# microsoft/Sora

Measured on AMD Instinct MI355X. Metric: IQ Msamples/s through 802.11a 54 Mbps RX PHY, higher is better.
Workload: dtype int16 IQ / u8 path metrics

## Files before the change

### sora_amd/csrc/dev_vit16.h

```cpp
#pragma once
#include <hip/hip_runtime.h>
#include "kernels.h"
#include "dev_viterbi.h"

namespace sora {
namespace {

template <int WIN, int LOOK> struct Geom16 {
    static constexpr int kMaxWalk = (WIN + LOOK + 7) / 8 + 2;
    static constexpr int P = kMaxWalk;
    static constexpr int kPathBytes = 40;
};

template <int WIN, int LOOK> struct Lds16 {
    uint16_t ring[Geom16<WIN, LOOK>::P][4][64];
    union {
        uint32_t udump[4][64];
        uint16_t ops[4][24][2];
        uint16_t ops2[2][4][24][2];
    };
    uint32_t path[8][Geom16<WIN, LOOK>::kPathBytes / 4];
};

constexpr unsigned kW[4] = { 0u, 21u, 42u, 63u };

__device__ __forceinline__ unsigned v_of_lane(unsigned l)
{
    const unsigned b0 = l & 1u, b1 = (l >> 1) & 1u, b2 = (l >> 2) & 1u, b3 = (l >> 3) & 1u;
    const unsigned c3 = b2, c1 = b3, c0 = b0 ^ c3, c2 = b1 ^ c3;
    return c0 | (c1 << 1) | (c2 << 2) | (c3 << 3);
}
__device__ __forceinline__ unsigned lane_of_v(unsigned v)
{
    const unsigned c0 = v & 1u, c1 = (v >> 1) & 1u, c2 = (v >> 2) & 1u, c3 = (v >> 3) & 1u;
    return c0 ^ (c2 << 1) ^ (c1 << 3) ^ (c3 ? 7u : 0u);
}
__device__ __forceinline__ unsigned rev6u(unsigned x) { return __brev(x) >> 26; }

template <int CTRL> __device__ __forceinline__ unsigned dppx(unsigned v) { return (unsigned)__builtin_amdgcn_update_dpp(0, (int)v, CTRL, 0xF, 0xF, true); }

__device__ __forceinline__ unsigned partner(unsigned v, int ph)
{
    switch (ph) {
    case 0: return dppx<0x140>(v);
    case 1: return dppx<0x1B>(v);
    case 2: return dppx<0x141>(v);
    case 3: return dppx<0x4E>(v);
    case 4: return dppx<0x128>(v);
    default: return dppx<0xB1>(v);
    }
}

struct Vit16 {
    unsigned U[4];
    unsigned MX[24];
    unsigned MY[6];
    unsigned sadr[3][4];
};

template <int WHICH, int P>
__device__ __forceinline__ void acs16(Vit16& V, int t24, unsigned a, unsigned b, unsigned pos512[3])
{
    const int ph = t24 % 6, k = t24 % 8;
    const unsigned Kp = (WHICH == 0 ? 14u : 7u) * kFld + (kOne << k);
    unsigned bm;
    if (WHICH == 0)      bm = (a ^ V.MX[t24]) + (b ^ V.MY[ph]);
    else if (WHICH == 1) bm = a ^ V.MX[t24];
    else                 bm = b ^ V.MX[t24];
    const unsigned bo = Kp - bm;
    const int rx = ph == 0 ? 2 : ph == 1 ? 1 : 0;
    unsigned N[4];
#pragma unroll
    for (int i = 0; i < 4; i++) {
        const unsigned X = V.U[i], Y = partner(V.U[i ^ rx], ph);
        const bool wb = (kW[i] >> (5 - ph)) & 1u;
        N[i] = wb ? pk_min16(X + bo, Y + bm) : pk_min16(X + bm, Y + bo);
    }
#pragma unroll
    for (int i = 0; i < 4; i++) V.U[i] = N[i];
    if (k == 7) {
        const int jb = t24 / 8;
#pragma unroll
        for (int i = 0; i < 4; i++) {
            const unsigned w = bank_word(V.U[i]);
            const unsigned addr = V.sadr[jb][i] + pos512[jb];
            asm volatile("ds_write_b16 %0, %1" : : "v"(addr), "v"(w) : "memory");
            V.U[i] &= 0xFE00FE00u;
        }
    }
}

__device__ __forceinline__ unsigned row_min_u32(unsigned v)
{
    v = min(v, dppx<0xB1>(v)); v = min(v, dppx<0x4E>(v)); v = min(v, dppx<0x141>(v)); v = min(v, dppx<0x128>(v));
    return v;
}
__device__ __forceinline__ unsigned row_pkmin(unsigned v)
{
    v = pk_min16(v, dppx<0xB1>(v)); v = pk_min16(v, dppx<0x4E>(v)); v = pk_min16(v, dppx<0x141>(v)); v = pk_min16(v, dppx<0x128>(v));
    return v;
}
__device__ __forceinline__ unsigned wave_min_u32(unsigned v) { return (unsigned)__builtin_amdgcn_readfirstlane((int)dpp_min_u32_wave(v)); }
__device__ __forceinline__ unsigned wave_max_u32(unsigned v) { return ~wave_min_u32(~v); }

template <int CR, int WIN, int LOOK, int BITS>
struct Forward16 {
    static constexpr int P = Geom16<WIN, LOOK>::P, GB = Puncture<CR>::GB, GS = Puncture<CR>::GS, CW = Puncture<CR>::CW;
    static constexpr int NV = Puncture<CR>::NV;
    struct Chunk { uint32_t v[CW]; };
    struct Raw { SoftRaw r[NV]; };

    Vit16 V;
    unsigned row, half;
    uint32_t my_j;
    SoftCursor<BITS, CW> cur[NV];
    uint32_t my_base;
    const uint8_t* soft;
    uint16_t* my_ops;
    const uint4* row_ops;
    uint32_t pos;
    unsigned pos512[3];
    uint32_t tr, nsteps;
    uint32_t next_thr;
    bool all_done;

    __device__ __forceinline__ void init(Lds16<WIN, LOOK>& S, const uint8_t* __restrict__ soft_, uint32_t my_soft_off, uint32_t my_first, uint32_t my_last, unsigned start,
                                         uint32_t nsteps_)
    {
        const unsigned lane = threadIdx.x & 63, l16 = lane & 15;
        row = lane >> 4; half = lane & 1u;
        const unsigned v0 = v_of_lane(l16);
        nsteps = nsteps_;
#pragma unroll
        for (int i = 0; i < 4; i++) V.U[i] = (v0 ^ kW[i]) == 0 ? 0u : start;
        const unsigned ring_base = (unsigned)(uintptr_t)&S.ring[0][0][0];
#pragma unroll
        for (int jb = 0; jb < 3; jb++)
#pragma unroll
            for (int i = 0; i < 4; i++) V.sadr[jb][i] = ring_base + ((row * 64u + rev6u(rol6(v0 ^ kW[i], jb == 0 ? 2 : jb == 1 ? 4 : 0))) << 1);
#pragma unroll
        for (int t = 0; t < 24; t++) {
            const int ph = t % 6, k = t % 8;
            const unsigned n = rol6(v0, ph + 1);
            const bool vb = (v0 >> (5 - ph)) & 1u;
            const unsigned ma = (__popc(n & 0155) & 1) ? 7u * kFld : 0u, mb = (__popc(n & 0117) & 1) ? 7u * kFld : 0u;
            const unsigned mx = Puncture<CR>::which_of(ph) == 2 ? mb : ma;
            V.MX[t] = vb ? ((mx ^ (7u * kFld)) | (kOne << k)) : mx;
            if (t < 6) V.MY[t] = vb ? (mb ^ (7u * kFld)) : mb;
        }
        tr = 0; pos = 0;
        my_j = l16 >> 1;
#pragma unroll
        for (int v = 0; v < NV; v++) cur[v].init(my_soft_off, my_first + my_j + 8u * v, my_last);
        my_base = my_soft_off + my_first + my_j;
        soft = soft_;
        my_ops = &S.ops[row][my_j][half];
        row_ops = reinterpret_cast<const uint4*>(&S.ops[row][0][0]);
        set_row_pos();
        clear_ops(S);
    }
    __device__ __forceinline__ bool going() const { return tr < nsteps && !all_done; }

    __device__ __forceinline__ void normalize()
    {
        const unsigned m = row_pkmin(pk_min16(pk_min16(V.U[0], V.U[1]), pk_min16(V.U[2], V.U[3])));
#pragma unroll
        for (int i = 0; i < 4; i++) V.U[i] -= m;
    }
    static __device__ __forceinline__ uint32_t pos_of(uint32_t p, int jb) { const uint32_t q = p + 512u * (uint32_t)jb; return min(q, q - 512u * (uint32_t)P); }
    __device__ __forceinline__ void set_row_pos()
    {
        pos512[0] = pos; pos512[1] = pos_of(pos, 1); pos512[2] = pos_of(pos512[1], 1);
    }
    __device__ __forceinline__ void end_row() { pos = pos_of(pos512[2], 1); set_row_pos(); }
    __device__ __forceinline__ Raw fetch(uint32_t c) const
    {
        Raw R;
#pragma unroll
        for (int v = 0; v < NV; v++) R.r[v] = cur[v].fetch(soft, c);
        return R;
    }
    __device__ __forceinline__ void put(const Raw& R, uint16_t* mine) const
    {
#pragma unroll
        for (int v = 0; v < NV; v++) soft_put(mine + 16 * v, cur[v], R.r[v]);
    }
    __device__ __forceinline__ void clear_ops(Lds16<WIN, LOOK>& S) const
    {
        if constexpr (BITS == kSoftScaled) {
            static_assert(sizeof(S.ops2) == 3 * 64 * 4, "three dwords per lane");
            uint32_t* z = reinterpret_cast<uint32_t*>(&S.ops2[0][0][0][0]) + (threadIdx.x & 63);
            z[0] = 0u; z[64] = 0u; z[128] = 0u;
            lds_fence();
        }
    }
    __device__ __forceinline__ uint32_t fast_base(uint32_t c0) const { return my_base + c0 * (uint32_t)CW; }
    template <int DC> __device__ __forceinline__ Raw fetch_at(uint32_t p) const
    {
        static_assert(BITS == kSoftScaled, "one byte per value");
        Raw R;
#pragma unroll
        for (int v = 0; v < NV; v++) { R.r[v].sh = 0; R.r[v].w = soft[(size_t)p + (size_t)(DC * CW + 8 * v)]; }
        return R;
    }
    static __device__ __forceinline__ Chunk get(const uint4* table)
    {
        Chunk K;
#pragma unroll
        for (int i = 0; i < (CW + 3) / 4; i++) {
            const uint4 x = table[i];
            K.v[4 * i] = x.x; K.v[4 * i + 1] = x.y;
            if (4 * i + 2 < CW) { K.v[4 * i + 2] = x.z; K.v[4 * i + 3] = x.w; }
        }
        return K;
    }
    __device__ __forceinline__ Chunk unpack(const Raw& R) const
    {
        put(R, my_ops);
        lds_fence();
        const Chunk K = get(row_ops);
        lds_fence();
        return K;
    }
    __device__ __forceinline__ void group(const Chunk& K, int h, int i0)
    {
        const int k0 = i0 / GS * GB, t24 = 12 * h + i0;
        acs16<0, P>(V, t24, K.v[k0], K.v[k0 + 1], pos512);
        if (CR != 0) acs16<1, P>(V, t24 + 1, K.v[k0 + 2], 0, pos512);
        if (CR == 2) acs16<2, P>(V, t24 + 2, 0, K.v[k0 + 3], pos512);
        if ((t24 + GS) % 8 == 0) normalize();
    }
    __device__ __forceinline__ void fast_chunk(const Chunk& K, int h)
    {
#pragma unroll
        for (int g = 0; g < 12 / GS; g++) group(K, h, g * GS);
        tr += 12;
    }
    template <typename CHECK> __device__ __forceinline__ void slow_chunk(const Chunk& K, int h, CHECK& check)
    {
#pragma unroll
        for (int g = 0; g < 12 / GS; g++) {
            if (going()) {
                group(K, h, g * GS);
                tr += GS;
                check(12 * h + g * GS + GS - 1);
            }
        }
    }
    template <typename CHECK> __device__ __forceinline__ void chunk(const Chunk& K, int h, CHECK& check)
    {
        if (tr + 12 <= nsteps && next_thr > tr + 12) fast_chunk(K, h); else slow_chunk(K, h, check);
    }
};

template <int WIN, int LOOK, bool LANE_OB = false>
__device__ __noinline__ void trace16(unsigned lds_off, unsigned U0, unsigned U1, unsigned U2, unsigned U3, uint32_t tr_, uint32_t ob_, uint32_t pj_, uint32_t k_,
                                     uint32_t my_cnt, uint8_t* my_out)
{
    using G = Geom16<WIN, LOOK>;
    constexpr int P = G::P, K = G::kMaxWalk;
    constexpr int NR = K - 1, NF = NR / 4, NW = K / 4 + 1;
    static_assert(NR % 4 == 0 || NR % 4 == 2, "the walk's words are packed in pairs");
    static_assert(NW * 4 <= G::kPathBytes && NW >= WIN / 32 + 1, "the stream's registers hold a window and fit Lds16::path");
    typedef __attribute__((address_space(3))) Lds16<WIN, LOOK> lds_t;
    typedef __attribute__((address_space(3))) const uint16_t lds_u16;
    lds_t& S = *(lds_t*)(uintptr_t)lds_off;
    auto uni = [](uint32_t v) { return (uint32_t)__builtin_amdgcn_readfirstlane((int)v); };
    const uint32_t tr = uni(tr_), ob = LANE_OB ? ob_ : uni(ob_), pj = uni(pj_), k = uni(k_);
    const unsigned lane = threadIdx.x & 63, row = lane >> 4, l16 = lane & 15, half = lane & 1u;
    const unsigned v0 = v_of_lane(l16);
    const unsigned U[4] = { U0, U1, U2, U3 };
    const uint32_t j = (tr - 1) >> 3, nn = tr - 8u * j, m_lo = ob >> 3;
    const unsigned rowbase = (unsigned)(uintptr_t)&S.ring[0][row][0], sh = 8u * half;
    auto ring_j = [&](unsigned idx) -> unsigned { return *(lds_u16*)(uintptr_t)(rowbase + pj + (idx << 1)); };
#pragma unroll
    for (int i = 0; i < 4; i++) S.udump[i][lane] = U[i];
    lds_fence();
    unsigned key[2] = { 0xFFFFFFFFu, 0xFFFFFFFFu };
#pragma unroll
    for (int i = 0; i < 4; i++) {
        const unsigned st = rol6(v0 ^ kW[i], tr);
        unsigned lastA, lastB;
        if (k == 7) { const unsigned w = ring_j(rev6u(st)); lastA = (w >> 7) & 1u; lastB = (w >> 15) & 1u; }
        else { lastA = (U[i] >> k) & 1u; lastB = (U[i] >> (17 + k)) & 1u; }
        const unsigned mA = ((U[i] & 0xFFFFu) >> 9 << 1) | lastA, mB = (U[i] >> 25 << 1) | lastB;
        key[0] = min(key[0], (mA << 8) | (st << 2)); key[1] = min(key[1], (mB << 8) | (st << 2));
    }
    const unsigned kA = row_min_u32(key[0]), kB = row_min_u32(key[1]);
    const unsigned st = ((half ? kB : kA) >> 2) & 0x3Fu;
    const unsigned s0 = rol6(st, 6u - tr % 6u);
    const unsigned b4 = (s0 >> 4) & 1u, b5 = (s0 >> 5) & 1u;
    const unsigned ri = b4 | (b5 << 1);
    const unsigned sl = lane_of_v((s0 ^ (b4 ? 21u : 0u) ^ (b5 ? 42u : 0u)) & 15u);
    const unsigned Ust = S.udump[ri][row * 16u + sl];
    unsigned H;
    if (nn == 8) H = (ring_j(rev6u(st)) >> sh) & 0xFFu;
    else H = ((Ust >> (17u * half)) & 0xFFu) & ((1u << nn) - 1u);
    unsigned q = rev6u(((st >> nn) | rev6u(H & 0x3Fu)) & 0x3Fu);
    unsigned pr[NR / 2];
    uint32_t p = pj;
#pragma unroll
    for (int i = 1; i < K; i++) {
        uint32_t d;
        p = __builtin_sub_overflow(p, 512u, &d) ? 512u * (uint32_t)(P - 1) : d;
        unsigned base = rowbase + p;
        asm volatile("" : "+v"(base));
        const unsigned raw = *(lds_u16*)(uintptr_t)(base + (q << 1));
        q = __builtin_amdgcn_ubfe(raw, sh, 6u);
        const int s = K - 1 - i;
        if (s & 1) pr[s >> 1] = raw << 16; else pr[s >> 1] |= raw;
    }
    unsigned R[NW];
    const unsigned sel = 0x06040200u + 0x01010101u * half;
#pragma unroll
    for (int w = 0; w < NF; w++) R[w] = __builtin_amdgcn_perm(pr[2 * w + 1], pr[2 * w], sel);
    if (NR % 4 == 0) R[NF] = H;
    else R[NF] = __builtin_amdgcn_perm(H, pr[2 * NF], 0x0C040200u + 0x00000101u * half);
    const uint32_t sfirst = (uint32_t)(K - 1) - (j - m_lo);
    bool fast = !LANE_OB;
    if (!LANE_OB) {
        const bool whole = my_cnt == (uint32_t)WIN && sfirst == 1u && (((uintptr_t)my_out + m_lo) & 3u) == 0;
        fast = __ballot(!(whole || my_cnt == 0)) == 0;
    }
    if (fast) {
        if (my_cnt != 0 && l16 < 2) {
            uint32_t* o = reinterpret_cast<uint32_t*>(my_out + m_lo);
#pragma unroll
            for (int dw = 0; dw < WIN / 32; dw++) o[dw] = __builtin_amdgcn_alignbit(R[dw + 1], R[dw], 14);
        }
    } else {
        __attribute__((address_space(3))) uint32_t* pw = S.path[row * 2u + half];
        if (l16 < 2) {
#pragma unroll
            for (int w = 0; w < NW; w++) pw[w] = R[w];
        }
        lds_fence();
        __attribute__((address_space(3))) const uint8_t* pth = (__attribute__((address_space(3))) const uint8_t*)pw;
        const uint32_t nbytes = my_cnt >> 3;
        for (uint32_t z = l16 >> 1; z < nbytes; z += 8) {
            const uint32_t sb = sfirst + z;
            my_out[m_lo + z] = (uint8_t)(((unsigned)pth[sb] >> 6) | (((unsigned)pth[sb + 1] & 0x3Fu) << 2));
        }
    }
    lds_fence();
}

}
}
```

### sora_amd/csrc/k_vit16.hip

```cpp
#include <hip/hip_runtime.h>

#include "dev_vit16.h"

namespace sora {

namespace {

template <int CR, int WIN, int LOOK, int BITS>
__device__ __forceinline__ void forward16(Lds16<WIN, LOOK>& S, const uint8_t* __restrict__ soft, uint32_t my_soft_off, uint32_t my_nsoft,
                                          uint32_t nstepsA, uint32_t nstepsB, uint32_t my_tr_end, bool my_valid, uint8_t* my_out)
{
    using F16 = Forward16<CR, WIN, LOOK, BITS>;
    using Chunk = typename F16::Chunk;
    using Raw = typename F16::Raw;
    constexpr int GS = F16::GS;
    F16 F;
    F.init(S, soft, my_soft_off, 0, max(my_nsoft, 1u) - 1u, 0x18u * kFld, wave_max_u32(max(nstepsA, nstepsB)));

    uint32_t ob = 0;
    bool my_done = !my_valid;

    auto trace = [&](uint32_t my_cnt, int t24_last) {
        trace16<WIN, LOOK>((unsigned)(uintptr_t)&S, F.V.U[0], F.V.U[1], F.V.U[2], F.V.U[3], F.tr, ob, F16::pos_of(F.pos, t24_last / 8), (uint32_t)(t24_last % 8), my_cnt, my_out);
    };
    auto next_event = [&]() -> uint32_t {
        const uint32_t mine = my_done ? kNever : my_tr_end;
        return min(ob + (uint32_t)(WIN + LOOK + 6), wave_min_u32(mine));
    };
    F.next_thr = next_event();
    F.all_done = wave_min_u32(my_done ? 1u : 0u) != 0u;
    auto check = [&](int t24_last) {
        if (F.tr >= F.next_thr) {
            const bool partial = F.tr >= ob + (uint32_t)(WIN + LOOK + 6);
            uint32_t cnt = 0;
            if (!my_done) {
                if (F.tr >= my_tr_end) { cnt = my_tr_end - ob - 6; my_done = true; }
                else if (partial) cnt = WIN;
            }
            if (wave_max_u32(cnt) != 0u) { trace(cnt, t24_last); F.clear_ops(S); }
            if (partial) ob += WIN;
            F.next_thr = next_event();
            F.all_done = wave_min_u32(my_done ? 1u : 0u) != 0u;
        }
    };

    uint16_t* my_ops2[2] = { &S.ops2[0][F.row][F.my_j][F.half], &S.ops2[1][F.row][F.my_j][F.half] };
    const uint4* row_ops2[2] = { reinterpret_cast<const uint4*>(&S.ops2[0][F.row][0][0]), reinterpret_cast<const uint4*>(&S.ops2[1][F.row][0][0]) };
    auto stage = [&](const Raw& R, int t) { F.put(R, my_ops2[t]); };
    auto collect = [&](int t) -> Chunk { lds_fence(); return F16::get(row_ops2[t]); };
    auto fast_chunk_mid = [&](const Chunk& K, int h, Chunk& Knext, int tnext) {
#pragma unroll
        for (int g = 0; g < 12 / GS; g++) {
            if (g == (12 / GS) / 2) Knext = collect(tnext);
            F.group(K, h, g * GS);
        }
        F.tr += 12;
    };

    uint32_t c = 0;
    Raw b0 = F.fetch(0), b1 = F.fetch(1), b2, b3;
    while (F.going()) {
        const uint32_t lim = min(F.nsteps, F.next_thr - 1);
        uint32_t rows = lim > F.tr ? (lim - F.tr) / 24 : 0;
        if (rows >= 2) {
            Chunk Ka, Kb;
            b2 = F.fetch(c + 2);
            stage(b0, 0); Ka = collect(0); lds_fence();
            if constexpr (BITS == kSoftScaled) {
                uint32_t p = F.fast_base(c);
                for (; rows >= 2; rows -= 2) {
                    b3 = F.template fetch_at<3>(p); stage(b1, 1); fast_chunk_mid(Ka, 0, Kb, 1);
                    b0 = F.template fetch_at<4>(p); stage(b2, 0); fast_chunk_mid(Kb, 1, Ka, 0);
                    F.end_row();
                    b1 = F.template fetch_at<5>(p); stage(b3, 1); fast_chunk_mid(Ka, 0, Kb, 1);
                    b2 = F.template fetch_at<6>(p); stage(b0, 0); fast_chunk_mid(Kb, 1, Ka, 0);
                    F.end_row();
                    c += 4; p += 4u * (uint32_t)F16::CW;
                }
            } else {
                for (; rows >= 2; rows -= 2) {
                    b3 = F.fetch(c + 3); stage(b1, 1); fast_chunk_mid(Ka, 0, Kb, 1);
                    b0 = F.fetch(c + 4); stage(b2, 0); fast_chunk_mid(Kb, 1, Ka, 0);
                    F.end_row();
                    b1 = F.fetch(c + 5); stage(b3, 1); fast_chunk_mid(Ka, 0, Kb, 1);
                    b2 = F.fetch(c + 6); stage(b0, 0); fast_chunk_mid(Kb, 1, Ka, 0);
                    F.end_row();
                    c += 4;
                }
            }
            lds_fence();
        }
        if (!(F.tr < F.nsteps)) break;
        b2 = F.fetch(c + 2);
        if (rows) F.fast_chunk(F.unpack(b0), 0); else F.chunk(F.unpack(b0), 0, check);
        if (!F.going()) break;
        b3 = F.fetch(c + 3);
        if (rows) F.fast_chunk(F.unpack(b1), 1); else F.chunk(F.unpack(b1), 1, check);
        F.end_row();
        b0 = b2; b1 = b3;
        c += 2;
    }
}

template <int WIN, int LOOK, int BITS>
__device__ __forceinline__ void viterbi16_body(const VitJob* __restrict__ jobs, const uint32_t* __restrict__ njobs3, uint32_t njobs_single, uint32_t stride,
                                               const uint8_t* __restrict__ soft, uint8_t* __restrict__ out)
{
    __shared__ Lds16<WIN, LOOK> S;
    uint32_t n[3] = { njobs_single, 0, 0 };
    if (njobs3) { n[0] = njobs3[0]; n[1] = njobs3[1]; n[2] = njobs3[2]; }
    uint32_t w = uni(blockIdx.x), list = 0;
    while (list < 3 && w >= (n[list] + 7) / 8) { w -= (n[list] + 7) / 8; list++; }
    if (list >= 3) return;
    const uint32_t njobs = uni(n[list]);
    jobs += (size_t)list * stride;
    const unsigned lane = threadIdx.x & 63, row = lane >> 4, half = lane & 1u;
    const uint32_t fa = 8u * w + 2u * row, fb = fa + 1u;
    const bool hasA = fa < njobs, hasB = fb < njobs;
    const VitJob& GA = jobs[hasA ? fa : 8u * w];
    const VitJob& GBj = jobs[hasB ? fb : (hasA ? fa : 8u * w)];
    const uint32_t code_rate = uni(jobs[8u * w].code_rate);
    const uint32_t gsd = code_rate == 0 ? 2u : code_rate == 2 ? 4u : 3u, gss = code_rate == 0 ? 1u : code_rate == 2 ? 3u : 2u;
    const uint32_t nstepsA = hasA ? GA.nsoft / gsd * gss : 0u, nstepsB = hasB ? GBj.nsoft / gsd * gss : 0u;
    const VitJob& Mine = half ? GBj : GA;
    const bool my_valid = half ? hasB : hasA;
    const uint32_t my_tr_end = Mine.length * 8u + 16u + 6u;
    uint8_t* my_out = out + Mine.out_off;
    if (code_rate == 0)      forward16<0, WIN, LOOK, BITS>(S, soft, Mine.soft_off, Mine.nsoft, nstepsA, nstepsB, my_tr_end, my_valid, my_out);
    else if (code_rate == 1) forward16<1, WIN, LOOK, BITS>(S, soft, Mine.soft_off, Mine.nsoft, nstepsA, nstepsB, my_tr_end, my_valid, my_out);
    else                     forward16<2, WIN, LOOK, BITS>(S, soft, Mine.soft_off, Mine.nsoft, nstepsA, nstepsB, my_tr_end, my_valid, my_out);
}

}

__global__ void __launch_bounds__(64) k_viterbi16(const VitJob* __restrict__ jobs, const uint32_t* __restrict__ njobs3, uint32_t njobs_single, uint32_t stride,
        const uint8_t* __restrict__ soft, uint8_t* __restrict__ out)
{ viterbi16_body<256, 24, kSoftScaled>(jobs, njobs3, njobs_single, stride, soft, out); }
__global__ void __launch_bounds__(64) k_viterbi16_p3(const VitJob* __restrict__ jobs, const uint32_t* __restrict__ njobs3, uint32_t njobs_single, uint32_t stride,
        const uint8_t* __restrict__ soft, uint8_t* __restrict__ out)
{ viterbi16_body<256, 24, 3>(jobs, njobs3, njobs_single, stride, soft, out); }
__global__ void __launch_bounds__(64) k_viterbi16_11n(const VitJob* __restrict__ jobs, const uint32_t* __restrict__ njobs3, uint32_t njobs_single,
        uint32_t stride, const uint8_t* __restrict__ soft, uint8_t* __restrict__ out)
{ viterbi16_body<192, 36, 8>(jobs, njobs3, njobs_single, stride, soft, out); }

}
```

### sora_amd/csrc/rx_types.h

```cpp
#pragma once
#include <stdint.h>

namespace sora {

struct CapDesc {
    uint64_t offset;
    uint32_t nsamples;
    uint32_t capture_id;
    uint32_t slot_base;
    uint32_t nslots;
};

struct FrameRow {
    uint32_t capture;
    uint32_t start_sample;
    uint32_t end_sample;
    uint32_t error_code;
    uint32_t rate_kbps;
    uint16_t length, nsym;
    uint16_t code_rate, nbpsc;
    uint32_t slot0;
    uint32_t crc32;
    int16_t  cfo_est;
    int16_t  cfo_comp, sfo_comp, cfo_tracker, sfo_tracker;
    uint16_t valid;
    uint32_t data_start;
    uint32_t pad[3];
};

struct FrameCtx {
    uint32_t freq[64];
    uint32_t chan[64];
};

struct VitJob {
    uint32_t soft_off;
    uint32_t nsoft;
    uint32_t length;
    uint32_t dec_off;
    uint32_t out_off;
    uint32_t valid;
    uint32_t code_rate;
    uint32_t soft_bits;
};

constexpr int kWinWarm = 144;
constexpr int kWinVecBytes = 256;
constexpr unsigned kWinStatBanks = 64;

struct TrackRec {
    int16_t cfo_comp, sfo_comp;
    int16_t avg, del;
};

struct JobRef { uint32_t list, idx; bool ok; };
__host__ __device__ inline JobRef locate_job(uint32_t g, const uint32_t* njobs)
{
    JobRef r; r.ok = true;
    const uint32_t n0 = njobs[0], n1 = njobs[1], n2 = njobs[2];
    if (g < n0) { r.list = 0; r.idx = g; }
    else if (g < n0 + n1) { r.list = 1; r.idx = g - n0; }
    else if (g < n0 + n1 + n2) { r.list = 2; r.idx = g - n0 - n1; }
    else { r.list = 0; r.idx = 0; r.ok = false; }
    return r;
}

constexpr int kSoftPerSlot = 288;
constexpr int kSoftBytesPerSlot = 288;
constexpr int kSoftSlack = 64;
constexpr int kSoftScaled = 9;
constexpr int kSoftPad = 66 * 1024;
static_assert(kSoftPad >= 65568 + 7 * 24 + 16 + kSoftSlack, "the pad holds a maximal stream and the look-ahead");
constexpr int kOutPerSlot  = 32;

constexpr uint32_t E_FRAME_OK = 0x00000001u, E_PLCP_HEADER_FAIL = 0x80000005u, E_CRC32_FAIL = 0x80000006u,
                   E_CS_TIMEOUT = 0x80000007u,
                   E_INTERNAL_TIMEOUT = 0x8000F001u;

}
```

Before: 56640.

## Distribute soft bits by DPP row broadcast instead of LDS staging in Viterbi

For the one-byte soft path, each lane now loads a dword of soft bits directly from global memory. Lanes swap bytes with a DPP quad permute, then each ACS step pulls its branch-metric operand from the owning lane with a DPP row broadcast. This removes the LDS put/fence/get staging and the clearing of the ops buffer from the hot trellis loop. The cost is extra permute and broadcast instructions per ACS step, and a larger look-ahead pad requirement.

```diff
diff --git a/sora_amd/csrc/dev_vit16.h b/sora_amd/csrc/dev_vit16.h
--- a/sora_amd/csrc/dev_vit16.h
+++ b/sora_amd/csrc/dev_vit16.h
@@ -38,6 +38,19 @@
 __device__ __forceinline__ unsigned rev6u(unsigned x) { return __brev(x) >> 26; }
 
 template <int CTRL> __device__ __forceinline__ unsigned dppx(unsigned v) { return (unsigned)__builtin_amdgcn_update_dpp(0, (int)v, CTRL, 0xF, 0xF, true); }
+__device__ __forceinline__ unsigned row_bcast(unsigned v, int n)
+{
+    switch (n) {
+    case 0: return dppx<0x150>(v);
+    case 2: return dppx<0x152>(v);
+    case 4: return dppx<0x154>(v);
+    case 6: return dppx<0x156>(v);
+    case 8: return dppx<0x158>(v);
+    case 10: return dppx<0x15A>(v);
+    case 12: return dppx<0x15C>(v);
+    default: return dppx<0x15E>(v);
+    }
+}
 
 __device__ __forceinline__ unsigned partner(unsigned v, int ph)
 {
@@ -103,12 +116,26 @@
 __device__ __forceinline__ unsigned wave_min_u32(unsigned v) { return (unsigned)__builtin_amdgcn_readfirstlane((int)dpp_min_u32_wave(v)); }
 __device__ __forceinline__ unsigned wave_max_u32(unsigned v) { return ~wave_min_u32(~v); }
 
-template <int CR, int WIN, int LOOK, int BITS>
+template <int CR, int WIN, int LOOK, int BITS, bool BCAST = false>
 struct Forward16 {
     static constexpr int P = Geom16<WIN, LOOK>::P, GB = Puncture<CR>::GB, GS = Puncture<CR>::GS, CW = Puncture<CR>::CW;
     static constexpr int NV = Puncture<CR>::NV;
-    struct Chunk { uint32_t v[CW]; };
+    static constexpr int RB = 2 * CW, RD = RB / 4, NS = (RD + 7) / 8;
+    static_assert(!BCAST || (BITS == kSoftScaled && RB % 4 == 0), "one byte per value, rows of whole dwords");
+    struct Chunk {
+        uint32_t v[CW];
+        __device__ __forceinline__ unsigned op(int, int k) const { return v[k]; }
+    };
     struct Raw { SoftRaw r[NV]; };
+    struct RawRow { uint32_t d[NS]; };
+    struct Row {
+        uint32_t r[NS][4];
+        __device__ __forceinline__ unsigned op(int h, int k) const
+        {
+            const int kk = h * CW + k;
+            return row_bcast(r[kk >> 5][kk & 3], 2 * ((kk >> 2) & 7));
+        }
+    };
 
     Vit16 V;
     unsigned row, half;
@@ -152,12 +179,12 @@
         my_j = l16 >> 1;
 #pragma unroll
         for (int v = 0; v < NV; v++) cur[v].init(my_soft_off, my_first + my_j + 8u * v, my_last);
-        my_base = my_soft_off + my_first + my_j;
+        my_base = BCAST ? my_soft_off + 4u * my_j : my_soft_off + my_first + my_j;
         soft = soft_;
         my_ops = &S.ops[row][my_j][half];
         row_ops = reinterpret_cast<const uint4*>(&S.ops[row][0][0]);
         set_row_pos();
-        clear_ops(S);
+        if constexpr (!BCAST) clear_ops(S);
     }
     __device__ __forceinline__ bool going() const { return tr < nsteps && !all_done; }
 
@@ -194,15 +221,6 @@
             lds_fence();
         }
     }
-    __device__ __forceinline__ uint32_t fast_base(uint32_t c0) const { return my_base + c0 * (uint32_t)CW; }
-    template <int DC> __device__ __forceinline__ Raw fetch_at(uint32_t p) const
-    {
-        static_assert(BITS == kSoftScaled, "one byte per value");
-        Raw R;
-#pragma unroll
-        for (int v = 0; v < NV; v++) { R.r[v].sh = 0; R.r[v].w = soft[(size_t)p + (size_t)(DC * CW + 8 * v)]; }
-        return R;
-    }
     static __device__ __forceinline__ Chunk get(const uint4* table)
     {
         Chunk K;
@@ -222,21 +240,40 @@
         lds_fence();
         return K;
     }
-    __device__ __forceinline__ void group(const Chunk& K, int h, int i0)
+    __device__ __forceinline__ uint32_t row_base(uint32_t row_index) const { return my_base + row_index * (uint32_t)RB; }
+    template <int DR> __device__ __forceinline__ RawRow fetch_row(uint32_t p) const
+    {
+        RawRow R;
+#pragma unroll
+        for (int s = 0; s < NS; s++) R.d[s] = *reinterpret_cast<const uint32_t*>(soft + ((size_t)p + (size_t)(DR * RB + 32 * s)));
+        return R;
+    }
+    static __device__ __forceinline__ Row assemble(const RawRow& R)
+    {
+        Row K;
+#pragma unroll
+        for (int s = 0; s < NS; s++) {
+            const unsigned mine = R.d[s], other = dppx<0xB1>(mine);
+#pragma unroll
+            for (int r = 0; r < 4; r++) K.r[s][r] = __builtin_amdgcn_perm(other, mine, 0x000C000Cu | ((unsigned)r << 8) | ((unsigned)(4 + r) << 24));
+        }
+        return K;
+    }
+    template <typename OPS> __device__ __forceinline__ void group(const OPS& K, int h, int i0)
     {
         const int k0 = i0 / GS * GB, t24 = 12 * h + i0;
-        acs16<0, P>(V, t24, K.v[k0], K.v[k0 + 1], pos512);
-        if (CR != 0) acs16<1, P>(V, t24 + 1, K.v[k0 + 2], 0, pos512);
-        if (CR == 2) acs16<2, P>(V, t24 + 2, 0, K.v[k0 + 3], pos512);
+        acs16<0, P>(V, t24, K.op(h, k0), K.op(h, k0 + 1), pos512);
+        if (CR != 0) acs16<1, P>(V, t24 + 1, K.op(h, k0 + 2), 0, pos512);
+        if (CR == 2) acs16<2, P>(V, t24 + 2, 0, K.op(h, k0 + 3), pos512);
         if ((t24 + GS) % 8 == 0) normalize();
     }
-    __device__ __forceinline__ void fast_chunk(const Chunk& K, int h)
+    template <typename OPS> __device__ __forceinline__ void fast_chunk(const OPS& K, int h)
     {
 #pragma unroll
         for (int g = 0; g < 12 / GS; g++) group(K, h, g * GS);
         tr += 12;
     }
-    template <typename CHECK> __device__ __forceinline__ void slow_chunk(const Chunk& K, int h, CHECK& check)
+    template <typename OPS, typename CHECK> __device__ __forceinline__ void slow_chunk(const OPS& K, int h, CHECK& check)
     {
 #pragma unroll
         for (int g = 0; g < 12 / GS; g++) {
@@ -247,7 +284,7 @@
             }
         }
     }
-    template <typename CHECK> __device__ __forceinline__ void chunk(const Chunk& K, int h, CHECK& check)
+    template <typename OPS, typename CHECK> __device__ __forceinline__ void chunk(const OPS& K, int h, CHECK& check)
     {
         if (tr + 12 <= nsteps && next_thr > tr + 12) fast_chunk(K, h); else slow_chunk(K, h, check);
     }
diff --git a/sora_amd/csrc/k_vit16.hip b/sora_amd/csrc/k_vit16.hip
--- a/sora_amd/csrc/k_vit16.hip
+++ b/sora_amd/csrc/k_vit16.hip
@@ -10,10 +10,8 @@
 __device__ __forceinline__ void forward16(Lds16<WIN, LOOK>& S, const uint8_t* __restrict__ soft, uint32_t my_soft_off, uint32_t my_nsoft,
                                           uint32_t nstepsA, uint32_t nstepsB, uint32_t my_tr_end, bool my_valid, uint8_t* my_out)
 {
-    using F16 = Forward16<CR, WIN, LOOK, BITS>;
-    using Chunk = typename F16::Chunk;
-    using Raw = typename F16::Raw;
-    constexpr int GS = F16::GS;
+    constexpr bool BCAST = BITS == kSoftScaled;
+    using F16 = Forward16<CR, WIN, LOOK, BITS, BCAST>;
     F16 F;
     F.init(S, soft, my_soft_off, 0, max(my_nsoft, 1u) - 1u, 0x18u * kFld, wave_max_u32(max(nstepsA, nstepsB)));
 
@@ -37,47 +35,68 @@
                 if (F.tr >= my_tr_end) { cnt = my_tr_end - ob - 6; my_done = true; }
                 else if (partial) cnt = WIN;
             }
-            if (wave_max_u32(cnt) != 0u) { trace(cnt, t24_last); F.clear_ops(S); }
+            if (wave_max_u32(cnt) != 0u) {
+                trace(cnt, t24_last);
+                if constexpr (!BCAST) F.clear_ops(S);
+            }
             if (partial) ob += WIN;
             F.next_thr = next_event();
             F.all_done = wave_min_u32(my_done ? 1u : 0u) != 0u;
         }
     };
 
-    uint16_t* my_ops2[2] = { &S.ops2[0][F.row][F.my_j][F.half], &S.ops2[1][F.row][F.my_j][F.half] };
-    const uint4* row_ops2[2] = { reinterpret_cast<const uint4*>(&S.ops2[0][F.row][0][0]), reinterpret_cast<const uint4*>(&S.ops2[1][F.row][0][0]) };
-    auto stage = [&](const Raw& R, int t) { F.put(R, my_ops2[t]); };
-    auto collect = [&](int t) -> Chunk { lds_fence(); return F16::get(row_ops2[t]); };
-    auto fast_chunk_mid = [&](const Chunk& K, int h, Chunk& Knext, int tnext) {
+    if constexpr (BCAST) {
+        using Row = typename F16::Row;
+        using RawRow = typename F16::RawRow;
+        uint32_t p = F.row_base(0);
+        RawRow b0 = F.template fetch_row<0>(p), b1 = F.template fetch_row<1>(p);
+        while (F.going()) {
+            const uint32_t lim = min(F.nsteps, F.next_thr - 1);
+            uint32_t rows = lim > F.tr ? (lim - F.tr) / 24 : 0;
+            for (; rows >= 2; rows -= 2) {
+                const Row Ka = F16::assemble(b0); b0 = F.template fetch_row<2>(p);
+                F.fast_chunk(Ka, 0); F.fast_chunk(Ka, 1);
+                F.end_row();
+                const Row Kb = F16::assemble(b1); b1 = F.template fetch_row<3>(p);
+                F.fast_chunk(Kb, 0); F.fast_chunk(Kb, 1);
+                F.end_row();
+                p += 2u * (uint32_t)F16::RB;
+            }
+            if (!(F.tr < F.nsteps)) break;
+            const Row K = F16::assemble(b0);
+            b0 = b1; b1 = F.template fetch_row<2>(p);
+            p += (uint32_t)F16::RB;
+            if (rows) F.fast_chunk(K, 0); else F.chunk(K, 0, check);
+            if (!F.going()) break;
+            if (rows) F.fast_chunk(K, 1); else F.chunk(K, 1, check);
+            F.end_row();
+        }
+    } else {
+        using Chunk = typename F16::Chunk;
+        using Raw = typename F16::Raw;
+        constexpr int GS = F16::GS;
+        uint16_t* my_ops2[2] = { &S.ops2[0][F.row][F.my_j][F.half], &S.ops2[1][F.row][F.my_j][F.half] };
+        const uint4* row_ops2[2] = { reinterpret_cast<const uint4*>(&S.ops2[0][F.row][0][0]), reinterpret_cast<const uint4*>(&S.ops2[1][F.row][0][0]) };
+        auto stage = [&](const Raw& R, int t) { F.put(R, my_ops2[t]); };
+        auto collect = [&](int t) -> Chunk { lds_fence(); return F16::get(row_ops2[t]); };
+        auto fast_chunk_mid = [&](const Chunk& K, int h, Chunk& Knext, int tnext) {
 #pragma unroll
-        for (int g = 0; g < 12 / GS; g++) {
-            if (g == (12 / GS) / 2) Knext = collect(tnext);
-            F.group(K, h, g * GS);
-        }
-        F.tr += 12;
-    };
+            for (int g = 0; g < 12 / GS; g++) {
+                if (g == (12 / GS) / 2) Knext = collect(tnext);
+                F.group(K, h, g * GS);
+            }
+            F.tr += 12;
+        };
 
-    uint32_t c = 0;
-    Raw b0 = F.fetch(0), b1 = F.fetch(1), b2, b3;
-    while (F.going()) {
-        const uint32_t lim = min(F.nsteps, F.next_thr - 1);
-        uint32_t rows = lim > F.tr ? (lim - F.tr) / 24 : 0;
-        if (rows >= 2) {
-            Chunk Ka, Kb;
-            b2 = F.fetch(c + 2);
-            stage(b0, 0); Ka = collect(0); lds_fence();
-            if constexpr (BITS == kSoftScaled) {
-                uint32_t p = F.fast_base(c);
-                for (; rows >= 2; rows -= 2) {
-                    b3 = F.template fetch_at<3>(p); stage(b1, 1); fast_chunk_mid(Ka, 0, Kb, 1);
-                    b0 = F.template fetch_at<4>(p); stage(b2, 0); fast_chunk_mid(Kb, 1, Ka, 0);
-                    F.end_row();
-                    b1 = F.template fetch_at<5>(p); stage(b3, 1); fast_chunk_mid(Ka, 0, Kb, 1);
-                    b2 = F.template fetch_at<6>(p); stage(b0, 0); fast_chunk_mid(Kb, 1, Ka, 0);
-                    F.end_row();
-                    c += 4; p += 4u * (uint32_t)F16::CW;
-                }
-            } else {
+        uint32_t c = 0;
+        Raw b0 = F.fetch(0), b1 = F.fetch(1), b2, b3;
+        while (F.going()) {
+            const uint32_t lim = min(F.nsteps, F.next_thr - 1);
+            uint32_t rows = lim > F.tr ? (lim - F.tr) / 24 : 0;
+            if (rows >= 2) {
+                Chunk Ka, Kb;
+                b2 = F.fetch(c + 2);
+                stage(b0, 0); Ka = collect(0); lds_fence();
                 for (; rows >= 2; rows -= 2) {
                     b3 = F.fetch(c + 3); stage(b1, 1); fast_chunk_mid(Ka, 0, Kb, 1);
                     b0 = F.fetch(c + 4); stage(b2, 0); fast_chunk_mid(Kb, 1, Ka, 0);
@@ -87,18 +106,18 @@
                     F.end_row();
                     c += 4;
                 }
+                lds_fence();
             }
-            lds_fence();
+            if (!(F.tr < F.nsteps)) break;
+            b2 = F.fetch(c + 2);
+            if (rows) F.fast_chunk(F.unpack(b0), 0); else F.chunk(F.unpack(b0), 0, check);
+            if (!F.going()) break;
+            b3 = F.fetch(c + 3);
+            if (rows) F.fast_chunk(F.unpack(b1), 1); else F.chunk(F.unpack(b1), 1, check);
+            F.end_row();
+            b0 = b2; b1 = b3;
+            c += 2;
         }
-        if (!(F.tr < F.nsteps)) break;
-        b2 = F.fetch(c + 2);
-        if (rows) F.fast_chunk(F.unpack(b0), 0); else F.chunk(F.unpack(b0), 0, check);
-        if (!F.going()) break;
-        b3 = F.fetch(c + 3);
-        if (rows) F.fast_chunk(F.unpack(b1), 1); else F.chunk(F.unpack(b1), 1, check);
-        F.end_row();
-        b0 = b2; b1 = b3;
-        c += 2;
     }
 }
 
diff --git a/sora_amd/csrc/rx_types.h b/sora_amd/csrc/rx_types.h
--- a/sora_amd/csrc/rx_types.h
+++ b/sora_amd/csrc/rx_types.h
@@ -70,7 +70,7 @@
 constexpr int kSoftSlack = 64;
 constexpr int kSoftScaled = 9;
 constexpr int kSoftPad = 66 * 1024;
-static_assert(kSoftPad >= 65568 + 7 * 24 + 16 + kSoftSlack, "the pad holds a maximal stream and the look-ahead");
+static_assert(kSoftPad >= 65568 + 48 + 2 * 48 + 64 + kSoftSlack, "the pad holds a maximal stream and the look-ahead");
 constexpr int kOutPerSlot  = 32;
 
 constexpr uint32_t E_FRAME_OK = 0x00000001u, E_PLCP_HEADER_FAIL = 0x80000005u, E_CRC32_FAIL = 0x80000006u,
```

Measured after the change: 56360. About the same (-0.5%).
